# antao97/SegGroup

Hardware: AMD Instinct MI355X
Metric: pseudo-label scenes/sec (150k pts, 1.5k segs) (higher is better)
Workload: dtype f32 (fp32 accumulate; operands split into 2 x fp16 pieces on v_mfma_f32_32x32x16_f16; kNN / FPS scores in exact fp32 order); 1 GPU; 64 distinct synthetic scenes per GPU per step, 150000 pts / 1500 segs each (BASELINE.json configs[2]; configs[1] = the same scene shape, single scene); mode=ins_infer, scenes_in_flight=112, engine=14 groups x 8 scenes per batched launch, weights=tests/golden/weights_g2.npz, parallelism=scene-parallel x1

## Files before the change

### include/seggroup_hip.h

```cpp
#ifndef SEGGROUP_HIP_H
#define SEGGROUP_HIP_H

#include <stddef.h>
#include <stdint.h>

#ifdef __cplusplus
extern "C" {
#endif

#define SG_OK          0
#define SG_EINVAL     -1
#define SG_EHIP       -2
#define SG_ENOMEM     -3
#define SG_ESTALL     -4
#define SG_EUNSUP     -5

#define SG_MODE_INS_INFER 0
#define SG_MODE_SEM_INFER 1

#define SG_NUM_LABEL_VECTORS 14
#define SG_RANGE_WORDS 256
#define SG_MAX_POINTS (1 << 20)

const char* sg_last_error(void);
// ... 64 lines not shown
                          const int32_t* d_seg_off, const int32_t* d_seg_chunk_off, const float* d_segbox,
                          const float* d_chunk_box, const int32_t* d_slot_of_pos, int k, int pos0, int32_t* d_knn, void* stream);
int sg_knn_seed_points(const int32_t* d_knn, const int32_t* d_members, int N, int k, int32_t* d_seed, void* stream);
int sg_cluster_knn_seeded(const float* d_sxyzw, const int32_t* d_smpos, int N, const int32_t* d_cl_off,
                          const int32_t* d_tile_cl, const int32_t* d_tile_lo, const int32_t* d_tile_hi, int T,
                          const int32_t* d_cl_seg_off, const int32_t* d_order, const int32_t* d_dst,
                          const int32_t* d_seg_off, const int32_t* d_seg_chunk_off, const float* d_segbox,
                          const float* d_chunk_box, const int32_t* d_slot_of_pos, const int32_t* d_seed,
                          const int32_t* d_seg_prevcl, const int32_t* d_members, const float* d_point_rec,
                          int k, int pos0, int32_t* d_knn, void* stream);

int sg_knn_chunk_table(const int32_t* d_order, const int32_t* d_dst, const int32_t* d_seg_off, const int32_t* d_seg_chunk_off,
                       const float* d_chunk_box, int S, const int32_t* d_slot_chunk0, float* d_cc, void* stream);
int sg_cluster_knn_2pass(const float* d_sxyzw, const int32_t* d_smpos, int N, const int32_t* d_cl_off,
                         const int32_t* d_tile_cl, const int32_t* d_tile_lo, const int32_t* d_tile_hi,
                         const int32_t* d_tile_chunk0, int T, const int32_t* d_cl_chunk_off, const float* d_cc,
                         int k, int pos0, int32_t* d_knn, void* stream);
int sg_cluster_knn_sorted_w(const float* d_sxyzw, const int32_t* d_smpos, int N, const int32_t* d_cl_off,
                            const int32_t* d_tile_cl, const int32_t* d_tile_lo, const int32_t* d_tile_hi, int T,
                            const int32_t* d_cl_seg_off, const int32_t* d_order, const int32_t* d_dst,
                            const int32_t* d_seg_off, const int32_t* d_seg_chunk_off, const float* d_segbox,
                            const float* d_chunk_box, const int32_t* d_slot_of_pos, int k, int pos0, int waves_per_tile,
                            int32_t* d_knn, void* stream);

size_t sg_edgeconv_ws_bytes(int N);
int sg_edgeconv_forward(const float* d_x9m, const int32_t* d_knn, int N, int k, int layers,
                        const float* d_w1, const float* d_g1, const float* d_b1,
                        const float* d_w2, const float* d_g2, const float* d_b2,
                        float* d_out, void* d_ws, size_t ws_bytes, void* stream);
int sg_edgeconv_forward_r(const float* d_x9m, const int32_t* d_knn, int N, int k, int layers, const float* d_w1, const float* d_g1,
                          const float* d_b1, const float* d_w2, const float* d_g2, const float* d_b2, float* d_out, void* d_ws,
                          size_t ws_bytes, unsigned int* d_range_bits, void* stream);
#define SG_EDGECONV_COMPILER_LOOP 1u
int sg_edgeconv_forward_x(const float* d_x9m, const int32_t* d_knn, int N, int k, int layers, const float* d_w1, const float* d_g1,
                          const float* d_b1, const float* d_w2, const float* d_g2, const float* d_b2, float* d_out, void* d_ws,
                          size_t ws_bytes, unsigned int* d_range_bits, unsigned int flags, void* stream);
int sg_edge_range(const float* d_x9m, int N, unsigned int* d_range_bits, void* stream);

size_t sg_gcn_ws_bytes(int S, int D, int E);
int sg_gcn_forward(const float* d_x, int S, int D, const int32_t* d_adj, int E,
                   const int32_t* d_rowptr, const int32_t* d_col, const int32_t* d_eid,
                   const float* d_w, float alpha, float* d_out, void* d_ws, size_t ws_bytes, void* stream);

int sg_export_labels(const int32_t* d_unmap, int V, const int32_t* d_seg_of_point, int N,
                     const int32_t* d_tables, int T, int S, int32_t* d_out, void* stream);

// ... 292 lines not shown
```

### seggroup_amd/csrc/kernels_knn_sorted.hip

```cpp
#include <cstdlib>


#include "engine_ctx.h"
#include "knn_device.h"
#include "sg_common.h"
#include "wave_ops.h"

namespace {

using namespace sgknn;

#ifdef SG_KNN_PROFILE
constexpr bool kKnnProfile = true;
#else
constexpr bool kKnnProfile = false;
#endif

constexpr int kChunkPts = 32;
constexpr int kQuadS = 4;

__device__ inline unsigned int spread10(unsigned int v);
__device__ inline unsigned int morton30(const float* __restrict__ r, const float* __restrict__ b) {
    const float e[3] = {b[3] - b[0], b[4] - b[1], b[5] - b[2]};
    const float emax = fmaxf(fmaxf(e[0], e[1]), e[2]);
// ... 475 lines not shown
    const sg::SlotCtx& c = cx[blockIdx.y];
    if ((int)blockIdx.x >= c.lay_nbig) return;
    const int i = c.lay_big[2 * blockIdx.x], r0 = c.lay_big[2 * blockIdx.x + 1];
    layer_layout_body(c.data, c.seg_points, c.seg_off, c.sperm, c.order, c.dst, c.cl, c.cl_mean, c.members, nullptr, c.cluster_of_pos,
                      c.slot_of_pos, c.x9m, c.sxyzw, c.smpos, c.point_rec, c.seed_id, c.ec_range, i, r0, r0 + sg::kLayoutPiece);
}

__global__ void k_knn_operands(const float* __restrict__ data, const int32_t* __restrict__ seg_points,
                               const int32_t* __restrict__ seg_off, const int32_t* __restrict__ sperm,
                               const int32_t* __restrict__ order, const int32_t* __restrict__ dst,
                               float4* __restrict__ sxyzw, int32_t* __restrict__ smpos) {
    const int i = blockIdx.x;
    const int s = order[i];
    const int lo = seg_off[s], n = seg_off[s + 1] - lo, d = dst[i];
    for (int r = threadIdx.x; r < n; r += blockDim.x) {
        const int ci = sperm[lo + r];
        const float* row = data + (size_t)seg_points[ci] * 6;
        const float x = row[0], y = row[1], z = row[2];
        sxyzw[d + r] = make_float4(x, y, z, (x * x + y * y) + z * z);
        smpos[d + r] = d + (ci - lo);
    }
}

__device__ unsigned long long g_knn5_stats[16];
#ifdef SG_KNN_SELFCHECK
__device__ unsigned long long g_knn_check[8 + 128];
#endif

template <int K, int kSlices, bool kSeeded>
__device__ __forceinline__ void cluster_knn_sorted_body(
    sg::gptr<const float4> sxyzw, sg::gptr<const int32_t> smpos, sg::gptr<const int32_t> cl_off,
    sg::gptr<const int32_t> tile_cl, sg::gptr<const int32_t> tile_lo, sg::gptr<const int32_t> tile_hi,
    sg::gptr<const int32_t> cl_seg_off, sg::gptr<const int32_t> order, sg::gptr<const int32_t> dst,
    sg::gptr<const int32_t> seg_off, sg::gptr<const int32_t> seg_chunk_off, sg::gptr<const float> segbox,
    sg::gptr<const float> chunk_box, sg::gptr<const int32_t> slot_of_pos, int pos0, sg::gptr<int32_t> knn, int dbg_arg,
    sg::gptr<const int32_t> seed, sg::gptr<const int32_t> seg_prevcl, sg::gptr<const int32_t> members,
    sg::gptr<const float4> point_rec, int t, sg::gptr<int32_t> seed_out = nullptr) {
    static_assert(!kSeeded || kSlices == 1, "seeding is built for one wave per tile");
    const int dbg = kKnnProfile ? dbg_arg : 0;
    constexpr int kBufS = kSlices == 1 ? 12 : 20;
    constexpr int kSlotBatch = kSlices == 1 ? 32 : 128;
    static_assert(kSlices == 1 || kBufS >= K, "the merge area aliases the append buffers");
    __shared__ float4 slab[kSlices][kChunkPts + kQuadS];
    __shared__ int slab_i[kSlices][kChunkPts + kQuadS];
    __shared__ unsigned long long buf[kBufS][64 * kSlices];
    __shared__ unsigned int thr_pub[kSlices][64];
    __shared__ unsigned int thr5_pub[kSlices][64];
    __shared__ __attribute__((aligned(16))) float chunkbox_lds[kSlices][kSlices == 1 ? 256 : 64];
    __shared__ int st_m[kSlotBatch], st_c0[kSlotBatch], st_d[kSlotBatch], st_pc[kSlotBatch];
    __shared__ __attribute__((aligned(16))) float st_box[kSlotBatch][8];
    const int c = tile_cl[t];
    const int clo = cl_off[c], n = cl_off[c + 1] - clo;
    const int tid = threadIdx.x, lane = tid & 63, wave = tid >> 6;
    const int q = tile_lo[t] + lane;
    const bool active = q < tile_hi[t];
    const int myrow = active ? smpos[q] : 0;
    if (n <= K) {
        if (active && wave == 0) {
            int lane_e = lane;
            asm volatile("" : "+v"(lane_e));
            const int row_e = smpos[tile_lo[t] + lane_e];
            const sg::gptr<int32_t> o = knn + (size_t)row_e * K;
#pragma unroll
            for (int j = 0; j < K; ++j) o[j] = j < n ? clo + j : pos0;
            if (seed_out) {
                const sg::gptr<int32_t> so = seed_out + (size_t)members[row_e] * K;
#pragma unroll
                for (int j = 0; j < K; ++j) so[j] = members[j < n ? clo + j : pos0];
            }
        }
        return;
    }
    float4 me = make_float4(0.f, 0.f, 0.f, 0.f);
    if (active) me = sxyzw[q];
    double kv[K];
#pragma unroll
    for (int j = 0; j < K; ++j) kv[j] = list_empty();
    double thr_l = active ? list_empty() : to_list(~0ull);
    int myprev = -1;
    if (kSeeded && active) {
        myprev = seg_prevcl[order[slot_of_pos[myrow]]];
        if (myprev >= 0) {
            const sg::gptr<const int32_t> sp = seed + (size_t)members[myrow] * K;
#pragma unroll
            for (int j = 0; j < K; ++j) {
                const float4 rec = point_rec[sp[j]];
                kv[j] = to_list(make_key(score4(me, make_float4(rec.x, rec.y, rec.z, (rec.x * rec.x + rec.y * rec.y) + rec.z * rec.z)),
                                         __float_as_int(rec.w) - clo));
            }
            thr_l = kv[K - 1];
#ifdef SG_KNN_SELFCHECK
            bool bad_ = false;
#pragma unroll
            for (int j = 0; j + 1 < K; ++j) bad_ |= from_list(kv[j]) <= from_list(kv[j + 1]);
            if (bad_ && atomicAdd(&g_knn_check[0], 1ull) == 0ull) {
                for (int j = 0; j < K; ++j) {
                    const float4 rec = point_rec[sp[j]];
                    g_knn_check[8 + j] = ((unsigned long long)(unsigned)sp[j] << 32) | (unsigned)(__float_as_int(rec.w) - clo);
                    g_knn_check[8 + 20 + j] = from_list(kv[j]);
                    const float again = score4(me, make_float4(rec.x, rec.y, rec.z, (rec.x * rec.x + rec.y * rec.y) + rec.z * rec.z));
// ... 82 lines not shown
        const double use_l = best_thr();
        if ((dbg & 32) && lane == 0) atomicAdd(&g_knn5_stats[6], 1ull);
        if (!__any(ok && list_key(box_score_bound(me, bx), 0) >= use_l)) return;
        if ((dbg & 32) && lane == 0) atomicAdd(&g_knn5_stats[5], 1ull);
        if (dbg & 16) ++dbg_scanned;
        __builtin_amdgcn_wave_barrier();
        if (lane < kChunkPts + kQuadS) {
            const bool in = lane < m;
            float4 cand = make_float4(0.f, 0.f, 0.f, INFINITY);
            if (in) cand = sxyzw[p0 + lane];
            cw[lane] = cand;
            ci[lane] = in ? smpos[p0 + lane] - clo : 0x7fffffff;
        }
        __builtin_amdgcn_wave_barrier();
        float fbound = score_bound(list_max(use_l, thr_l), ok);
        for (int i = 0; i < m; i += kQuadS) {
            float4 c4[kQuadS];
#pragma unroll
            for (int u = 0; u < kQuadS; ++u) c4[u] = cw[i + u];
            float sc4[kQuadS];
#pragma unroll
            for (int u = 0; u < kQuadS; ++u) sc4[u] = score4(me, c4[u]);
            static_assert(kQuadS == 4, "the group test below is written for four candidates");
            if (fmaxf(fmaxf(sc4[0], sc4[1]), fmaxf(sc4[2], sc4[3])) >= fbound) {
#pragma unroll
                for (int u = 0; u < kQuadS; ++u) {
                    if (sc4[u] >= fbound) {
                        const double key = list_key(sc4[u], ci[i + u]);
                        if (key > use_l && key > thr_l) {
                            buf[cnt][tid] = (unsigned long long)__double_as_longlong(key);
                            ++cnt;
                        }
                    }
                }
            }
            if (__any(cnt > kBufS - kQuadS)) {
                drain();
                fbound = score_bound(list_max(use_l, thr_l), ok);
            }
        }
    };
    const int so0 = cl_seg_off[c], nslots = cl_seg_off[c + 1] - so0;
    const int own = slot_of_pos[active ? myrow : smpos[tile_lo[t]]] - so0;
    const int own0 = __shfl(own, 0);
    auto slot_of = [&](int r) {
        int sl = own0 + r;
        if (sl >= nslots) sl -= nslots;
        return so0 + sl;
    };
    float* cbx = &chunkbox_lds[wave][0];
    float qlo[3] = {0.f, 0.f, 0.f}, qhi[3] = {0.f, 0.f, 0.f}, qw = 0.f;
    if (kSlices == 1) {
        const float4 m0 = active ? me : make_float4(sgw::bcast(me.x, 0), sgw::bcast(me.y, 0), sgw::bcast(me.z, 0), sgw::bcast(me.w, 0));
        qlo[0] = sgw::wave_min(m0.x); qlo[1] = sgw::wave_min(m0.y); qlo[2] = sgw::wave_min(m0.z);
        qhi[0] = sgw::wave_max(m0.x); qhi[1] = sgw::wave_max(m0.y); qhi[2] = sgw::wave_max(m0.z);
        qw = sgw::wave_max(m0.w);
    }
    auto ring_chunk = [](int start, int e, int nch, bool two_sided) {
        int ch = start + (two_sided ? ((e & 1) ? -((e + 1) >> 1) : (e >> 1)) : e);
        if (ch >= nch) ch -= nch;
        if (ch < 0) ch += nch;
        return ch;
    };
    auto scan_segment = [&](int sg_m, int sg_c0, int d, const float* sbox, int pc, int& item, int start, bool two_sided = false) {
        const int nch = (sg_m + kChunkPts - 1) / kChunkPts;
        const double use_l = best_thr();
        if (kSeeded) ok = pc < 0 || pc != myprev;
        if ((dbg & 32) && lane == 0 && wave == 0) atomicAdd(&g_knn5_stats[7], 1ull);
        if (!__any(ok && list_key(box_score_bound(me, sbox), 0) >= use_l)) { item += nch; return; }
        if constexpr (kSlices == 1) {
            for (int j0 = 0; j0 < nch; j0 += 32) {
                const int nb = min(32, nch - j0);
                const int mych = ring_chunk(start, min(j0 + lane, nch - 1), nch, two_sided);
                bool pass = lane < nb;
                float weakest = -INFINITY;
                if (nch > 16) {
                    const unsigned int o = list_score(best_thr());
                    float mine = INFINITY;
                    if (active && ok) mine = o < 0x00800000u ? -INFINITY : __uint_as_float((o & 0x80000000u) ? (o ^ 0x80000000u) : ~o);
                    weakest = sgw::wave_min(mine);
                }
                __builtin_amdgcn_wave_barrier();
                if (lane < nb) {
                    const sg::gptr<const float4> bp = (sg::gptr<const float4>)(chunk_box + (size_t)(sg_c0 + mych) * 8);
                    const float4 b0 = bp[0], b1 = bp[1];
                    reinterpret_cast<float4*>(cbx)[2 * lane] = b0;
                    reinterpret_cast<float4*>(cbx)[2 * lane + 1] = b1;
                    if (nch > 16) {
                        const float gx = fmaxf(fmaxf(b0.x - qhi[0], qlo[0] - b0.w), 0.f);
                        const float gy = fmaxf(fmaxf(b0.y - qhi[1], qlo[1] - b1.x), 0.f);
                        const float gz = fmaxf(fmaxf(b0.z - qhi[2], qlo[2] - b1.y), 0.f);
                        pass = -((gx * gx + gy * gy) + gz * gz) * 0.999999f + 9.6e-7f * (qw + b1.z) >= weakest;
                    }
                }
                __builtin_amdgcn_wave_barrier();
                unsigned long long live = __ballot(pass);
                while (live) {
                    const int j = __ffsll((unsigned long long)live) - 1;
                    live &= live - 1;
                    const int ch = ring_chunk(start, j0 + j, nch, two_sided);
                    scan_chunk(cbx + j * 8, d + ch * kChunkPts, min(kChunkPts, sg_m - ch * kChunkPts));
                }
            }
            item += nch;
            return;
        }
        for (int j0 = 0; j0 < nch; j0 += 8) {
            const int nb = min(8, nch - j0);
            __builtin_amdgcn_wave_barrier();
            if (lane < nb * 8) cbx[lane] = chunk_box[(size_t)(sg_c0 + j0) * 8 + lane];
            __builtin_amdgcn_wave_barrier();
// ... 24 lines not shown
            const int slot = slot_of(r0 + e), sg = order[slot];
            st_m[e] = seg_off[sg + 1] - seg_off[sg];
            st_c0[e] = seg_chunk_off[sg];
            st_d[e] = dst[slot];
            if (kSeeded) st_pc[e] = seg_prevcl[sg];
            const sg::gptr<const float4> bp = (sg::gptr<const float4>)(segbox + (size_t)sg * 8);
            reinterpret_cast<float4*>(&st_box[e][0])[0] = bp[0];
            reinterpret_cast<float4*>(&st_box[e][0])[1] = bp[1];
        }
        __syncthreads();
        for (int i = 0; i < nb; ++i) scan_segment(st_m[i], st_c0[i], st_d[i], &st_box[i][0], kSeeded ? st_pc[i] : -1, item, 0);
    }
    drain();
    const unsigned long long t3 = (dbg & 16) ? __builtin_readcyclecounter() : 0ull;
#ifdef SG_KNN_SELFCHECK
    if (kSeeded && active) {
        bool bad_ = false;
#pragma unroll
        for (int j = 0; j + 1 < K; ++j) bad_ |= from_list(kv[j]) <= from_list(kv[j + 1]);
        if (bad_) atomicAdd(&g_knn_check[1], 1ull);
    }
#endif
    if (kSlices == 1) {
        if (active) {
            int lane_o = lane;
            asm volatile("" : "+v"(lane_o));
            const int row_o = smpos[tile_lo[t] + lane_o];
            const sg::gptr<int32_t> o = knn + (size_t)row_o * K;
#pragma unroll
            for (int j = 0; j < K; ++j) o[j] = clo + list_index(kv[j]);
            if (seed_out) {
                const sg::gptr<int32_t> so = seed_out + (size_t)members[row_o] * K;
#pragma unroll
                for (int j = 0; j < K; ++j) so[j] = members[clo + list_index(kv[j])];
            }
        }
    } else {
        __syncthreads();
        unsigned long long* lists = &buf[0][0];
    #pragma unroll
        for (int j = 0; j < K; ++j) lists[((size_t)wave * K + j) * 64 + lane] = from_list(kv[j]);
        __syncthreads();
        if (wave == 0 && active) {
            int p[kSlices];
            unsigned long long h[kSlices];
    #pragma unroll
            for (int w = 0; w < kSlices; ++w) { p[w] = 0; h[w] = lists[((size_t)w * K) * 64 + lane]; }
            const sg::gptr<int32_t> o = knn + (size_t)myrow * K;
            for (int j = 0; j < K; ++j) {
                int bw = 0;
                unsigned long long bk = h[0];
    #pragma unroll
                for (int w = 1; w < kSlices; ++w) if (h[w] > bk) { bk = h[w]; bw = w; }
                o[j] = clo + key_index(bk);
    #pragma unroll
                for (int w = 0; w < kSlices; ++w)
                    if (w == bw) { ++p[w]; h[w] = p[w] < K ? lists[((size_t)w * K + p[w]) * 64 + lane] : 0ull; }
            }
        }
    }
    if ((dbg & 16) && lane == 0) {
        const unsigned long long t4 = __builtin_readcyclecounter();
        if (wave == 0) atomicAdd(&g_knn5_stats[0], 1ull);
        atomicAdd(&g_knn5_stats[1], t1 - t0);
        atomicAdd(&g_knn5_stats[2], t2 - t1);
        atomicAdd(&g_knn5_stats[3], t3 - t2);
        atomicAdd(&g_knn5_stats[4], t4 - t3);
        atomicMax(&g_knn5_stats[13], (min(t4 - t0, 0xffffffull) << 40) | ((unsigned long long)min(n >> 6, 0x3fff) << 26) |
                                     ((unsigned long long)min(nslots, 0xfff) << 14) | (unsigned long long)min(dbg_scanned, 0x3fff));
        if (n > 2048) { atomicAdd(&g_knn5_stats[14], t4 - t0); atomicAdd(&g_knn5_stats[15], 1ull); }
    }
}
template <int K, int kSlices, bool kSeeded = false>
__global__ __launch_bounds__(64 * kSlices, kSlices == 1 ? 4 : 1) void k_cluster_knn_sorted(
    const float4* __restrict__ sxyzw, const int32_t* __restrict__ smpos, const int32_t* __restrict__ cl_off,
    const int32_t* __restrict__ tile_cl, const int32_t* __restrict__ tile_lo, const int32_t* __restrict__ tile_hi,
    const int32_t* __restrict__ cl_seg_off, const int32_t* __restrict__ order, const int32_t* __restrict__ dst,
    const int32_t* __restrict__ seg_off, const int32_t* __restrict__ seg_chunk_off, const float* __restrict__ segbox,
    const float* __restrict__ chunk_box, const int32_t* __restrict__ slot_of_pos, int pos0, int32_t* __restrict__ knn, int dbg_arg,
    const int32_t* __restrict__ seed = nullptr, const int32_t* __restrict__ seg_prevcl = nullptr, const int32_t* __restrict__ members = nullptr,
    const float4* __restrict__ point_rec = nullptr) {
    using sg::as_global;
    cluster_knn_sorted_body<K, kSlices, kSeeded>(as_global(sxyzw), as_global(smpos), as_global(cl_off), as_global(tile_cl), as_global(tile_lo),
                                                 as_global(tile_hi), as_global(cl_seg_off), as_global(order), as_global(dst), as_global(seg_off),
                                                 as_global(seg_chunk_off), as_global(segbox), as_global(chunk_box), as_global(slot_of_pos), pos0,
                                                 as_global(knn), dbg_arg, as_global(seed), as_global(seg_prevcl), as_global(members),
                                                 as_global(point_rec), blockIdx.x);
}
template <int K, int kSlices, bool kSeeded>
__global__ __launch_bounds__(64 * kSlices, kSlices == 1 ? 4 : 1) void k_cluster_knn_sorted_b(const sg::SlotCtx* __restrict__ cx, int write_seed) {
    const sg::SlotCtx& c = cx[blockIdx.x];
    if ((int)blockIdx.y >= c.T) return;
    using sg::as_global;
    cluster_knn_sorted_body<K, kSlices, kSeeded>(as_global(c.sxyzw), as_global(c.smpos), as_global(c.cl_pt_off), as_global(c.tile_cl),
                                                 as_global(c.tile_lo), as_global(c.tile_hi), as_global(c.cl_seg_off), as_global(c.order),
                                                 as_global(c.dst), as_global(c.seg_off), as_global(c.seg_chunk_off), as_global(c.segbox),
                                                 as_global(c.chunk_box), as_global(c.slot_of_pos), c.pos0, as_global(c.knn), 0,
                                                 as_global(c.knn_seed), as_global(c.seg_prevcl), as_global(c.seed_id), as_global(c.point_rec),
                                                 blockIdx.y, kSlices == 1 && !kSeeded && write_seed ? as_global(c.knn_seed) : nullptr);
}


__global__ void k_knn_seed_points(const int32_t* __restrict__ knn, const int32_t* __restrict__ members, int N, int K,
                                  int32_t* __restrict__ seed) {
    const int i = blockIdx.x * blockDim.x + threadIdx.x;
    if (i >= N * K) return;
    seed[(size_t)members[i / K] * K + i % K] = members[knn[i]];
}
__global__ void k_knn_seed_points_b(const sg::SlotCtx* __restrict__ cx) {
    const sg::SlotCtx& c = cx[blockIdx.y];
    const int i = blockIdx.x * blockDim.x + threadIdx.x;
    if (i >= c.N * 20) return;
    c.knn_seed[(size_t)c.seed_id[i / 20] * 20 + i % 20] = c.seed_id[c.knn[i]];
}

template <int K>
__device__ inline void score_insert(float (&sv)[K], float x) {
#pragma unroll
    for (int j = K - 1; j > 0; --j) sv[j] = __builtin_amdgcn_fmed3f(sv[j - 1], sv[j], x);
    sv[0] = fmaxf(sv[0], x);
}

// ... 156 lines not shown
                 const unsigned long long key = make_key(sc, idx);
                 if (key > thr) {
                     buf[cnt][lane] = key;
                     ++cnt;
                 }
             },
             [&]() { return __any(cnt > kBuf2 - kQuadS - 1); }, drain);
    }
    if (active) {
        int32_t* o = knn + (size_t)myrow * K;
#pragma unroll
        for (int j = 0; j < K; ++j) o[j] = clo + key_index(kv[j]);
    }
    if ((dbg & 16) && lane == 0) {
        const unsigned long long t2 = __builtin_readcyclecounter();
        atomicAdd(&g_knn5_stats[0], 1ull);
        atomicAdd(&g_knn5_stats[1], t1 - t0);
        atomicAdd(&g_knn5_stats[3], t2 - t1);
    }
}

}

int sg::knn_variant_for(int T, int override) {
    if (override == 0 || override == 1 || override == 2 || override == 4 || override == 8) return override;
    return T >= 2048 ? 8 : T >= 1024 ? 2 : 4;
}

namespace sg {

bool sort_boxes_fits_lds(int max_seg) { return max_seg <= kSortCap; }

int b_sort_boxes(const SlotCtx* d_ctx, const BatchDims& bd, hipStream_t st, int which) {
    if (bd.nslots == 0 || bd.max_S == 0) return SG_OK;
    if (which & 1) k_segment_sort_boxes_b<<<dim3(bd.max_S, bd.nslots), 256, 0, st>>>(d_ctx);
    if ((which & 2) && bd.max_big > 0) {
        const int wins = sg::cdiv(bd.max_N, kWin);
        k_bigseg_box_b<<<dim3(bd.max_big * kBigPieces, bd.nslots), kPieceBlock, 0, st>>>(d_ctx);
        k_bigseg_keys_b<<<dim3(bd.max_big * kBigPieces, bd.nslots), kPieceBlock, 0, st>>>(d_ctx);
        k_bigseg_scatter_b<<<dim3(bd.max_big * kBigPieces, bd.nslots), kPieceBlock, 0, st>>>(d_ctx);
        k_bigseg_runs_b<<<dim3(wins, bd.nslots), kBigBlock, 0, st>>>(d_ctx);
        k_bigseg_boxes_b<<<dim3(wins, bd.nslots), 512, 0, st>>>(d_ctx);
    }
    SG_LAUNCH_CHECK();
    return SG_OK;
}

int b_layer_layout(const SlotCtx* d_ctx, const BatchDims& bd, hipStream_t st) {
    if (bd.nslots == 0 || bd.max_S == 0) return SG_OK;
    k_layer_layout_b<<<dim3(bd.max_S, bd.nslots), 256, 0, st>>>(d_ctx);
    if (bd.max_lay_big > 0) k_layer_layout_big_b<<<dim3(bd.max_lay_big, bd.nslots), 256, 0, st>>>(d_ctx);
    SG_LAUNCH_CHECK();
    return SG_OK;
}

int b_cluster_knn(const SlotCtx* d_ctx, const BatchDims& bd, int waves_per_tile, bool seeded, hipStream_t st, bool write_seed, bool* wrote_seed) {
    if (wrote_seed) *wrote_seed = false;
    if (bd.nslots == 0 || bd.max_T == 0) return SG_OK;
    if (bd.max_N > sgknn::kListMaxPoints) return sg::fail(SG_EUNSUP, "in-cluster kNN: %d points in a scene, the list keys carry 20 index bits (N <= %d)", bd.max_N, sgknn::kListMaxPoints);
    const dim3 grid(bd.nslots, bd.max_T);
    if (seeded) k_cluster_knn_sorted_b<20, 1, true><<<grid, 64, 0, st>>>(d_ctx, 0);
    else if (waves_per_tile == 1) {
        k_cluster_knn_sorted_b<20, 1, false><<<grid, 64, 0, st>>>(d_ctx, write_seed ? 1 : 0);
        if (wrote_seed) *wrote_seed = write_seed;
    } else if (waves_per_tile == 2) k_cluster_knn_sorted_b<20, 2, false><<<grid, 128, 0, st>>>(d_ctx, 0);
    else k_cluster_knn_sorted_b<20, 4, false><<<grid, 256, 0, st>>>(d_ctx, 0);
    SG_LAUNCH_CHECK();
    return SG_OK;
}

int b_knn_seed_points(const SlotCtx* d_ctx, const BatchDims& bd, hipStream_t st) {
    if (bd.nslots == 0 || bd.max_N == 0) return SG_OK;
    k_knn_seed_points_b<<<dim3(sg::cdiv((long long)bd.max_N * 20, 256), bd.nslots), 256, 0, st>>>(d_ctx);
    SG_LAUNCH_CHECK();
    return SG_OK;
}

}

#ifdef SG_KNN_PROFILE
static int g_knn5_dbg = getenv("SG_KNN_DEBUG") ? atoi(getenv("SG_KNN_DEBUG")) : 0;
#else
static constexpr int g_knn5_dbg = 0;
#endif

extern "C" {

#ifdef SG_KNN_PROFILE
int sg_debug_knn5_stats(unsigned long long* h_out) {
    SG_HIP(hipMemcpyFromSymbol(h_out, HIP_SYMBOL(g_knn5_stats), sizeof(unsigned long long) * 16));
    unsigned long long z[16] = {0};
    SG_HIP(hipMemcpyToSymbol(HIP_SYMBOL(g_knn5_stats), z, sizeof z));
    return SG_OK;
}
#endif

#ifdef SG_KNN_SELFCHECK
int sg_debug_knn_check(unsigned long long* h_out) {
    SG_HIP(hipMemcpyFromSymbol(h_out, HIP_SYMBOL(g_knn_check), sizeof(unsigned long long) * 136));
    unsigned long long z[136] = {0};
    SG_HIP(hipMemcpyToSymbol(HIP_SYMBOL(g_knn_check), z, sizeof z));
    return SG_OK;
}
#endif

size_t sg_segment_sort_ws_bytes(int N) { return sg::align_up((size_t)std::max(N, 1) * 16, 64) + bigseg_scratch_slots(std::max(N, 1)) * sizeof(BigScratch) + 64; }

int sg_layer_layout(const float* d_data, int N, const int32_t* d_seg_points, const int32_t* d_seg_off, const int32_t* d_sperm, int S,
                    const int32_t* d_order, const int32_t* d_dst, const int32_t* d_cl, const float* d_cl_mean, int32_t* d_members,
                    int32_t* d_pos_of_point, int32_t* d_cluster_of_pos, int32_t* d_slot_of_pos, float* d_x9m, float* d_sxyzw,
                    int32_t* d_smpos, float* d_point_rec, int32_t* d_seed_id, unsigned int* d_range_bits, void* stream) {
    SG_REQUIRE(N >= 0 && S >= 0 && d_sperm && d_cl_mean && d_members && d_pos_of_point && d_cluster_of_pos && d_slot_of_pos && d_x9m &&
                   d_sxyzw && d_smpos, "sg_layer_layout: bad arguments");
    if (S == 0) return SG_OK;
// ... 78 lines not shown
    SG_REQUIRE(N < (1 << 25), "sg_cluster_knn_2pass: sorted positions are packed in 25 bits (N < 2^25)");
    if (k != 20) return sg::fail(SG_EUNSUP, "sg_cluster_knn_2pass: only k == 20 is built (model.py:788,829), got %d", k);
    if (T == 0) return SG_OK;
    k_cluster_knn_2pass<20><<<T, 64, 0, sg::as_stream(stream)>>>(reinterpret_cast<const float4*>(d_sxyzw), d_smpos, d_cl_off, d_tile_cl,
                                                                 d_tile_lo, d_tile_hi, d_tile_chunk0, d_cl_chunk_off,
                                                                 reinterpret_cast<const float4*>(d_cc), pos0, d_knn, g_knn5_dbg);
    SG_LAUNCH_CHECK();
    return SG_OK;
}

int sg_cluster_knn_sorted_w(const float* d_sxyzw, const int32_t* d_smpos, int N, const int32_t* d_cl_off, const int32_t* d_tile_cl,
                            const int32_t* d_tile_lo, const int32_t* d_tile_hi, int T, const int32_t* d_cl_seg_off,
                            const int32_t* d_order, const int32_t* d_dst, const int32_t* d_seg_off, const int32_t* d_seg_chunk_off,
                            const float* d_segbox, const float* d_chunk_box, const int32_t* d_slot_of_pos, int k, int pos0,
                            int waves_per_tile, int32_t* d_knn, void* stream) {
    SG_REQUIRE(N >= 0 && T >= 0 && d_knn && d_sxyzw && d_smpos, "sg_cluster_knn_sorted: bad arguments");
    SG_REQUIRE(N <= sgknn::kListMaxPoints, "sg_cluster_knn_sorted: the list keys carry 20 index bits (N <= 2^20)");
    if (k != 20) return sg::fail(SG_EUNSUP, "sg_cluster_knn_sorted: only k == 20 is built (model.py:788,829), got %d", k);
    if (T == 0) return SG_OK;
    const int slices = (waves_per_tile == 1 || waves_per_tile == 2 || waves_per_tile == 4) ? waves_per_tile : (T >= 2048 ? 1 : T >= 1024 ? 2 : 4);
#define SG_KNN_LAUNCH(S)                                                                                                  \
    k_cluster_knn_sorted<20, S><<<T, 64 * S, 0, sg::as_stream(stream)>>>(                                                 \
        reinterpret_cast<const float4*>(d_sxyzw), d_smpos, d_cl_off, d_tile_cl, d_tile_lo, d_tile_hi, d_cl_seg_off, d_order, d_dst, \
        d_seg_off, d_seg_chunk_off, d_segbox, d_chunk_box, d_slot_of_pos, pos0, d_knn, g_knn5_dbg)
    if (slices == 1) SG_KNN_LAUNCH(1);
    else if (slices == 2) SG_KNN_LAUNCH(2);
    else SG_KNN_LAUNCH(4);
#undef SG_KNN_LAUNCH
    SG_LAUNCH_CHECK();
    return SG_OK;
}

int sg_cluster_knn_sorted(const float* d_sxyzw, const int32_t* d_smpos, int N, const int32_t* d_cl_off, const int32_t* d_tile_cl,
                          const int32_t* d_tile_lo, const int32_t* d_tile_hi, int T, const int32_t* d_cl_seg_off,
                          const int32_t* d_order, const int32_t* d_dst, const int32_t* d_seg_off, const int32_t* d_seg_chunk_off,
                          const float* d_segbox, const float* d_chunk_box, const int32_t* d_slot_of_pos, int k, int pos0,
                          int32_t* d_knn, void* stream) {
    return sg_cluster_knn_sorted_w(d_sxyzw, d_smpos, N, d_cl_off, d_tile_cl, d_tile_lo, d_tile_hi, T, d_cl_seg_off, d_order, d_dst, d_seg_off,
                                   d_seg_chunk_off, d_segbox, d_chunk_box, d_slot_of_pos, k, pos0, 0, d_knn, stream);
}

}
```

### seggroup_amd/csrc/knn_device.h

```cpp
#pragma once
#include <hip/hip_runtime.h>

namespace sgknn {

__device__ inline float score4(const float4& me, const float4& p) {
    const float tt = __builtin_fmaf(me.z, p.z, __builtin_fmaf(me.y, p.y, me.x * p.x));
    const float inner = -2.0f * tt;
    return ((-p.w) - inner) - me.w;
}

__device__ inline unsigned long long make_key(float score, int idx) {
    const unsigned int u = __float_as_uint(score);
    const unsigned int o = u ^ ((u >> 31) ? 0xffffffffu : 0x80000000u);
    return ((unsigned long long)o << 32) | (unsigned int)(0xffffffffu - (unsigned int)idx);
}
__device__ inline int key_index(unsigned long long key) { return (int)(0xffffffffu - (unsigned int)(key & 0xffffffffu)); }

__device__ __forceinline__ unsigned int sel_mask(unsigned int if_clear, unsigned int if_set, unsigned long long mask) {
    unsigned int r;
    asm("v_cndmask_b32_e64 %0, %1, %2, %3" : "=v"(r) : "v"(if_clear), "v"(if_set), "s"(mask));
    return r;
}
template <int K>
__device__ inline void key_insert(unsigned long long (&kv)[K], unsigned long long x) {
// ... 6 lines not shown
        const unsigned int pl = (unsigned int)kv[j - 1], ph = (unsigned int)(kv[j - 1] >> 32);
        const unsigned int ol = (unsigned int)kv[j], oh = (unsigned int)(kv[j] >> 32);
        const unsigned int tl = sel_mask(xl, pl, c[j - 1]), th = sel_mask(xh, ph, c[j - 1]);
        kv[j] = ((unsigned long long)sel_mask(oh, th, c[j]) << 32) | sel_mask(ol, tl, c[j]);
    }
    kv[0] = ((unsigned long long)sel_mask((unsigned int)(kv[0] >> 32), xh, c[0]) << 32) | sel_mask((unsigned int)kv[0], xl, c[0]);
}

constexpr int kListIndexBits = 20;
constexpr int kListMaxPoints = 1 << kListIndexBits;
__device__ __forceinline__ double list_empty() { return __hiloint2double(0x43300000, 0); }
__device__ __forceinline__ double to_list(unsigned long long key) {
    const unsigned int o = (unsigned int)(key >> 32), lo = (unsigned int)key;
    return __hiloint2double((int)(0x43300000u | (o >> 12)), (int)((o << 20) | (lo & 0xfffffu)));
}
__device__ __forceinline__ unsigned long long from_list(double d) {
    const unsigned int hi = (unsigned int)__double2hiint(d), lo = (unsigned int)__double2loint(d);
    return ((unsigned long long)((hi << 12) | (lo >> 20)) << 32) | (0xfff00000u | lo);
}
__device__ __forceinline__ double list_key(float score, int idx) {
    const unsigned int u = __float_as_uint(score);
    const unsigned int o = u ^ ((u >> 31) ? 0xffffffffu : 0x80000000u);
    return __hiloint2double((int)(0x43300000u | (o >> 12)), (int)((o << 20) | (~(unsigned int)idx & 0xfffffu)));
}
__device__ __forceinline__ unsigned int list_score(double d) {
    return __builtin_amdgcn_alignbit((unsigned int)__double2hiint(d), (unsigned int)__double2loint(d), 20);
}
__device__ __forceinline__ double list_floor(unsigned int o) {
    return __longlong_as_double(__double_as_longlong(__hiloint2double((int)(0x43300000u | (o >> 12)), (int)(o << 20))) - 1ll);
}
__device__ __forceinline__ int list_index(double d) { return (int)(0xfffffu - ((unsigned int)__double2loint(d) & 0xfffffu)); }
__device__ __forceinline__ double list_max(double a, double b) { double r; asm("v_max_f64 %0, %1, %2" : "=v"(r) : "v"(a), "v"(b)); return r; }
__device__ __forceinline__ double list_min(double a, double b) { double r; asm("v_min_f64 %0, %1, %2" : "=v"(r) : "v"(a), "v"(b)); return r; }
template <int K>
__device__ __forceinline__ void list_insert_l(double (&kv)[K], double x) {
#pragma unroll
    for (int j = K - 1; j > 0; --j) kv[j] = list_max(kv[j], list_min(kv[j - 1], x));
    kv[0] = list_max(kv[0], x);
}
template <int K>
__device__ __forceinline__ void list_insert(double (&kv)[K], unsigned long long key) {
    const double x = to_list(key);
#pragma unroll
    for (int j = K - 1; j > 0; --j) kv[j] = list_max(kv[j], list_min(kv[j - 1], x));
    kv[0] = list_max(kv[0], x);
}
// ... 40 lines not shown
```

### seggroup_amd/hip.py

```python
from __future__ import annotations

import contextlib
import ctypes as C
import os
from typing import Optional

_HERE = os.path.dirname(os.path.abspath(__file__))
LIB_PATH = os.environ.get("SEGGROUP_HIP_LIB") or os.path.join(_HERE, "libseggroup_hip.so")
HOST_LIB_OVERRIDE = os.environ.get("SEGGROUP_HIP_HOST_LIB")

SG_OK, SG_EINVAL, SG_EHIP, SG_ENOMEM, SG_ESTALL, SG_EUNSUP = 0, -1, -2, -3, -4, -5
MODE_INS_INFER, MODE_SEM_INFER = 0, 1
COLOUR_SEMANTIC, COLOUR_INSTANCE, COLOUR_SEGMENT, COLOUR_GROUPING = 0, 1, 2, 3
NUM_LABEL_VECTORS = 14
LABEL_NAMES = [f"layer_{l}.{k}" for l in (1, 2, 3, 4) for k in ("seg", "ins", "sem")] + ["final.ins", "final.sem"]

c_f32p = C.POINTER(C.c_float)
c_i32p = C.POINTER(C.c_int32)
c_i64p = C.POINTER(C.c_int64)
c_u8p = C.POINTER(C.c_uint8)
vp = C.c_void_p


class SgError(RuntimeError):
# ... 9 lines not shown

class Scene(C.Structure):
    _fields_ = [("N", C.c_int), ("S", C.c_int), ("E0", C.c_int), ("V", C.c_int),
                ("d_data", vp), ("d_adj", vp), ("d_seg_of_point", vp), ("d_seg_points", vp), ("d_seg_off", vp),
                ("d_unmap", vp), ("d_gt", vp),
                ("h_seg_first", vp), ("h_seg_size", vp), ("h_seg_ins", vp), ("h_seg_sem", vp), ("h_seg_of_vertex", vp)]


class Result(C.Structure):
    _fields_ = [("h_labels", vp), ("iou_sem", C.c_float * 80), ("iou_ins", C.c_float * 80), ("acc", C.c_float * 4),
                ("trace", C.c_int32 * 5), ("stalled", C.c_int32), ("used_fallback", C.c_int32), ("h_tables", vp)]


class Classifier(C.Structure):
    _fields_ = [(n, vp) for n in ("w1", "gamma", "beta", "w2", "b2")]


class Debug(C.Structure):
    _fields_ = [("d_samples1", vp), ("d_feat1", vp), ("d_pointfeat", vp * 2), ("d_knn", vp * 2), ("d_members", vp * 2),
                ("h_gcn", vp * 2), ("h_dist", vp * 3), ("h_adj", vp * 4), ("n_adj", C.c_int32 * 4),
                ("h_feat5", vp), ("h_ins5", vp), ("h_sem5", vp), ("n5", C.c_int32), ("tape", vp), ("d_cat", vp * 2)]


_I, _Z = C.c_int, C.c_size_t
SIGNATURES = {
    "sg_last_error": (C.c_char_p, []),
    "sg_version": (_I, []),
    "sg_device_count": (_I, []),
    "sg_selftest_wave_ops": (_I, [C.POINTER(C.c_int), vp]),
    "sg_selftest_list_insert": (_I, [C.POINTER(C.c_int), vp]),
    "sg_contract_ws_bytes": (_Z, [_I]),
    "sg_contract_point_edges": (_I, [vp, _I, vp, _I, _I, vp, _I, vp, vp, _Z, vp]),
    "sg_gather_members": (_I, [vp, vp, _I, vp, vp, vp, vp, vp, vp, vp, vp]),
    "sg_fps_ws_bytes": (_Z, [_I]),
    "sg_fps_sample": (_I, [vp, _I, _I, vp, vp, _I, _I, _I, _I, vp, vp, vp, _Z, vp]),
    "sg_mlp1_ws_bytes": (_Z, [_I]),
    "sg_mlp1_forward": (_I, [vp, _I, vp, vp, vp, vp, _I, vp, _Z, vp]),
    "sg_edge_distance": (_I, [vp, _I, _I, vp, _I, vp, vp]),
    "sg_group_max_rows": (_I, [vp, _I, _I, vp, vp, _I, vp, _I, vp]),
    "sg_segment_max": (_I, [vp, _I, _I, vp, vp, _I, _I, vp]),
    "sg_center_ws_bytes": (_Z, [_I, _I]),
    "sg_center_clusters": (_I, [vp, _I, vp, vp, _I, vp, vp, vp, _I, vp, vp, vp, vp, _Z, vp]),
    "sg_cluster_knn": (_I, [vp, _I, vp, vp, vp, vp, _I, _I, _I, vp, vp]),
    "sg_segment_boxes": (_I, [vp, vp, vp, _I, vp, vp]),
    "sg_cluster_knn_pruned": (_I, [vp, _I, vp, vp, vp, vp, _I, vp, vp, vp, vp, vp, vp, _I, _I, vp, vp]),
    "sg_segment_sort_ws_bytes": (_Z, [_I]),
    "sg_knn_operands": (_I, [vp, vp, vp, vp, _I, vp, vp, vp, vp, vp]),
    "sg_cluster_knn_sorted": (_I, [vp, vp, _I, vp, vp, vp, vp, _I, vp, vp, vp, vp, vp, vp, vp, vp, _I, _I, vp, vp]),
    "sg_segment_sort_boxes": (_I, [vp, _I, vp, vp, vp, _I, vp, _I, vp, vp, vp, vp, vp, _Z, vp]),
    "sg_layer_layout": (_I, [vp, _I, vp, vp, vp, _I, vp, vp, vp, vp, vp, vp, vp, vp, vp, vp, vp, vp, vp, vp, vp]),
    "sg_cluster_knn_sorted_w": (_I, [vp, vp, _I, vp, vp, vp, vp, _I, vp, vp, vp, vp, vp, vp, vp, vp, _I, _I, _I, vp, vp]),
    "sg_knn_seed_points": (_I, [vp, vp, _I, _I, vp, vp]),
    "sg_cluster_knn_seeded": (_I, [vp, vp, _I, vp, vp, vp, vp, _I, vp, vp, vp, vp, vp, vp, vp, vp, vp, vp, vp, vp, _I, _I, vp, vp]),
    "sg_knn_chunk_table": (_I, [vp, vp, vp, vp, vp, _I, vp, vp, vp]),
    "sg_cluster_knn_2pass": (_I, [vp, vp, _I, vp, vp, vp, vp, vp, _I, vp, vp, _I, _I, vp, vp]),
    "sg_nearest_point_ws_bytes": (_Z, [_I]),
    "sg_nearest_point": (_I, [vp, _I, vp, _I, _I, vp, vp, _Z, vp]),
    "sg_prep_sample_ws_bytes": (_Z, [_I, _I]),
    "sg_prep_sample_points": (_I, [vp, vp, _I, vp, _I, vp, vp, C.POINTER(C.c_int), vp, _Z, vp]),
    "sg_pointcloud_adjacency_ws_bytes": (_Z, [_I, _I]),
    "sg_pointcloud_adjacency": (_I, [vp, _I, _I, _I, vp, C.POINTER(C.c_int), vp, _Z, vp]),
    "sg_mesh_adjacency_ws_bytes": (_Z, [_I]),
    "sg_mesh_adjacency": (_I, [vp, _I, vp, _I, vp, C.POINTER(C.c_int), vp, C.POINTER(C.c_int), vp, _Z, vp]),
    "sg_segment_lists_ws_bytes": (_Z, [_I, _I]),
    "sg_segment_lists": (_I, [vp, _I, vp, _I, vp, vp, vp, C.POINTER(C.c_int), vp, _Z, vp]),
    "sg_write_seg_json": (_I, [C.c_char_p, vp, vp, _I, _I]),
    "sg_train_tail_ws_bytes": (_Z, [_I, _I]),
    "sg_train_tail_forward": (_I, [vp, _I, vp, _I, vp, vp, vp, vp, vp, vp, _Z, vp]),
    "sg_train_tail_backward": (_I, [_I, _I, vp, vp, vp, C.c_float, vp, vp, vp, vp, vp, vp, vp, _Z, vp]),
    "sg_group_mean_rows": (_I, [vp, _I, _I, vp, vp, _I, vp, _I, vp]),
    "sg_fps_general_ws_bytes": (C.c_size_t, [_I]),
    "sg_fps_general": (_I, [vp, _I, _I, _I, _I, _I, vp, vp, vp, C.c_size_t, vp]),
    "sg_knn_general": (_I, [vp, _I, _I, _I, _I, vp, vp]),
    "sg_group_max_rows_backward": (_I, [vp, _I, _I, vp, vp, _I, vp, _I, vp, _I, vp]),
# ... 127 lines not shown
            _runtime = C.CDLL(c, mode=C.RTLD_GLOBAL)
            return _runtime
        except OSError as e:
            err = e
    raise RuntimeError(f"no HIP runtime (libamdhip64.so) could be loaded: {err}")


def lib() -> C.CDLL:
    global _lib
    if _lib is None:
        path = HOST_LIB_OVERRIDE or LIB_PATH
        if not os.path.exists(path):
            raise RuntimeError(
                f"{path} is missing: build it with `python -c 'import __graft_entry__ as g; g.build()'` "
                "(or `make -C seggroup_amd/csrc`).  The SegGroup hot path has no CPU fallback.")
        _load_hip_runtime()
        l = C.CDLL(path)
        for name, (res, args) in SIGNATURES.items():
            try:
                fn = getattr(l, name)
            except AttributeError:
                if HOST_LIB_OVERRIDE:
                    continue
                raise
            fn.restype = res
            fn.argtypes = args
        _lib = l
    return _lib


_roctx = None


@contextlib.contextmanager
def roctx_range(name: str):
    global _roctx
    if not os.environ.get("SG_ROCTX"):
        yield
        return
    if _roctx is None:
        _roctx = False
        for cand in ("librocprofiler-sdk-roctx.so", "/opt/rocm/lib/librocprofiler-sdk-roctx.so", "libroctx64.so"):
            try:
                _roctx = C.CDLL(cand, mode=C.RTLD_GLOBAL)
                break
            except OSError:
# ... 29 lines not shown
```

Before: 3502 scenes/s.

## Add dense brute-force kNN path for small clusters, skipping chunk pruning

For clusters with at most a threshold number of points (default 256, env-tunable), the single-wave kNN kernel now scans every candidate in groups of twelve through a shared-memory slab and merges straight into the top-20 list, bypassing the segment/chunk box pruning machinery. The query tile bounding box is now computed lazily and stored in LDS only when chunk pruning actually needs it. This targets the bookkeeping overhead of the pruned search on small clusters, at the cost of exhaustive distance work for clusters near the threshold. A standalone entry point and profiling counters are also added.

Result: no change. 3519 scenes/s, median of 3 (+0.5%).

```diff
diff --git a/include/seggroup_hip.h b/include/seggroup_hip.h
--- a/include/seggroup_hip.h
+++ b/include/seggroup_hip.h
@@ -110,6 +110,13 @@
                             const int32_t* d_seg_off, const int32_t* d_seg_chunk_off, const float* d_segbox,
                             const float* d_chunk_box, const int32_t* d_slot_of_pos, int k, int pos0, int waves_per_tile,
                             int32_t* d_knn, void* stream);
+int sg_knn_dense_max(void);
+int sg_cluster_knn_sorted_d(const float* d_sxyzw, const int32_t* d_smpos, int N, const int32_t* d_cl_off,
+                            const int32_t* d_tile_cl, const int32_t* d_tile_lo, const int32_t* d_tile_hi, int T,
+                            const int32_t* d_cl_seg_off, const int32_t* d_order, const int32_t* d_dst,
+                            const int32_t* d_seg_off, const int32_t* d_seg_chunk_off, const float* d_segbox,
+                            const float* d_chunk_box, const int32_t* d_slot_of_pos, int k, int pos0, int dense_max,
+                            const int32_t* d_members, int32_t* d_seed_out, int32_t* d_knn, void* stream);
 
 size_t sg_edgeconv_ws_bytes(int N);
 int sg_edgeconv_forward(const float* d_x9m, const int32_t* d_knn, int N, int k, int layers,
diff --git a/seggroup_amd/csrc/kernels_knn_sorted.hip b/seggroup_amd/csrc/kernels_knn_sorted.hip
--- a/seggroup_amd/csrc/kernels_knn_sorted.hip
+++ b/seggroup_amd/csrc/kernels_knn_sorted.hip
@@ -521,7 +521,8 @@
     }
 }
 
-__device__ unsigned long long g_knn5_stats[16];
+constexpr int kKnnStats = 24;
+__device__ unsigned long long g_knn5_stats[kKnnStats];
 #ifdef SG_KNN_SELFCHECK
 __device__ unsigned long long g_knn_check[8 + 128];
 #endif
@@ -534,7 +535,7 @@
     sg::gptr<const int32_t> seg_off, sg::gptr<const int32_t> seg_chunk_off, sg::gptr<const float> segbox,
     sg::gptr<const float> chunk_box, sg::gptr<const int32_t> slot_of_pos, int pos0, sg::gptr<int32_t> knn, int dbg_arg,
     sg::gptr<const int32_t> seed, sg::gptr<const int32_t> seg_prevcl, sg::gptr<const int32_t> members,
-    sg::gptr<const float4> point_rec, int t, sg::gptr<int32_t> seed_out = nullptr) {
+    sg::gptr<const float4> point_rec, int t, sg::gptr<int32_t> seed_out = nullptr, int dense_max = 0) {
     static_assert(!kSeeded || kSlices == 1, "seeding is built for one wave per tile");
     const int dbg = kKnnProfile ? dbg_arg : 0;
     constexpr int kBufS = kSlices == 1 ? 12 : 20;
@@ -548,6 +549,7 @@
     __shared__ __attribute__((aligned(16))) float chunkbox_lds[kSlices][kSlices == 1 ? 256 : 64];
     __shared__ int st_m[kSlotBatch], st_c0[kSlotBatch], st_d[kSlotBatch], st_pc[kSlotBatch];
     __shared__ __attribute__((aligned(16))) float st_box[kSlotBatch][8];
+    __shared__ __attribute__((aligned(16))) float qbox_lds[8];
     const int c = tile_cl[t];
     const int clo = cl_off[c], n = cl_off[c + 1] - clo;
     const int tid = threadIdx.x, lane = tid & 63, wave = tid >> 6;
@@ -575,6 +577,54 @@
     double kv[K];
 #pragma unroll
     for (int j = 0; j < K; ++j) kv[j] = list_empty();
+    auto emit_rows = [&]() {
+        if (active) {
+            int lane_o = lane;
+            asm volatile("" : "+v"(lane_o));
+            const int row_o = smpos[tile_lo[t] + lane_o];
+            const sg::gptr<int32_t> o = knn + (size_t)row_o * K;
+#pragma unroll
+            for (int j = 0; j < K; ++j) o[j] = clo + list_index(kv[j]);
+            if (seed_out) {
+                const sg::gptr<int32_t> so = seed_out + (size_t)members[row_o] * K;
+#pragma unroll
+                for (int j = 0; j < K; ++j) so[j] = members[clo + list_index(kv[j])];
+            }
+        }
+    };
+    if constexpr (K == 20 && kSlices == 1 && !kSeeded) {
+        if (n <= dense_max) {
+            static_assert(kChunkPts + kQuadS == 36, "the dense path fills the slab with three groups of twelve");
+            float4* dw = slab[0];
+            int* di = slab_i[0];
+            const int ngroups = (n + 11) / 12;
+            if ((dbg & 32) && lane == 0) { atomicAdd(&g_knn5_stats[16], 1ull); atomicAdd(&g_knn5_stats[17], (unsigned long long)ngroups); }
+            int r12 = 0;
+            for (int g = 0; g < ngroups; ++g) {
+                if (r12 == 0) {
+                    __builtin_amdgcn_wave_barrier();
+                    if (lane < kChunkPts + kQuadS) {
+                        const int p = g * 12 + lane;
+                        float4 cand = make_float4(0.f, 0.f, 0.f, INFINITY);
+                        int bits = 0;
+                        if (p < n) { cand = sxyzw[clo + p]; bits = ~(smpos[clo + p] - clo) & 0xfffff; }
+                        dw[lane] = cand;
+                        di[lane] = bits;
+                    }
+                    __builtin_amdgcn_wave_barrier();
+                }
+                const int left = n - g * 12;
+                double b[12];
+#pragma unroll
+                for (int u = 0; u < 12; ++u)
+                    b[u] = list_key_bits(score4(me, dw[r12 + u]), (unsigned int)di[r12 + u], u < left ? 0xffffffffu : 0u);
+                list_merge12(kv, b);
+                r12 = r12 == 24 ? 0 : r12 + 12;
+            }
+            emit_rows();
+            return;
+        }
+    }
     double thr_l = active ? list_empty() : to_list(~0ull);
     int myprev = -1;
     if (kSeeded && active) {
@@ -703,6 +753,12 @@
 #pragma unroll
             for (int u = 0; u < kQuadS; ++u) sc4[u] = score4(me, c4[u]);
             static_assert(kQuadS == 4, "the group test below is written for four candidates");
+            if (dbg & 32) {
+                int took = 0;
+#pragma unroll
+                for (int u = 0; u < kQuadS; ++u) took += (i + u < m && __any(sc4[u] >= fbound)) ? 1 : 0;
+                if (lane == 0) { atomicAdd(&g_knn5_stats[18], (unsigned long long)min(kQuadS, m - i)); atomicAdd(&g_knn5_stats[19], (unsigned long long)took); }
+            }
             if (fmaxf(fmaxf(sc4[0], sc4[1]), fmaxf(sc4[2], sc4[3])) >= fbound) {
 #pragma unroll
                 for (int u = 0; u < kQuadS; ++u) {
@@ -730,13 +786,18 @@
         return so0 + sl;
     };
     float* cbx = &chunkbox_lds[wave][0];
-    float qlo[3] = {0.f, 0.f, 0.f}, qhi[3] = {0.f, 0.f, 0.f}, qw = 0.f;
-    if (kSlices == 1) {
+    bool have_qbox = false;
+    auto tile_qbox = [&]() {
         const float4 m0 = active ? me : make_float4(sgw::bcast(me.x, 0), sgw::bcast(me.y, 0), sgw::bcast(me.z, 0), sgw::bcast(me.w, 0));
-        qlo[0] = sgw::wave_min(m0.x); qlo[1] = sgw::wave_min(m0.y); qlo[2] = sgw::wave_min(m0.z);
-        qhi[0] = sgw::wave_max(m0.x); qhi[1] = sgw::wave_max(m0.y); qhi[2] = sgw::wave_max(m0.z);
-        qw = sgw::wave_max(m0.w);
-    }
+        const float lo0 = sgw::wave_min(m0.x), lo1 = sgw::wave_min(m0.y), lo2 = sgw::wave_min(m0.z);
+        const float hi0 = sgw::wave_max(m0.x), hi1 = sgw::wave_max(m0.y), hi2 = sgw::wave_max(m0.z);
+        const float w = sgw::wave_max(m0.w);
+        if (lane == 0) {
+            reinterpret_cast<float4*>(qbox_lds)[0] = make_float4(lo0, lo1, lo2, w);
+            reinterpret_cast<float4*>(qbox_lds)[1] = make_float4(hi0, hi1, hi2, 0.f);
+        }
+        have_qbox = true;
+    };
     auto ring_chunk = [](int start, int e, int nch, bool two_sided) {
         int ch = start + (two_sided ? ((e & 1) ? -((e + 1) >> 1) : (e >> 1)) : e);
         if (ch >= nch) ch -= nch;
@@ -756,6 +817,7 @@
                 bool pass = lane < nb;
                 float weakest = -INFINITY;
                 if (nch > 16) {
+                    if (!have_qbox) tile_qbox();
                     const unsigned int o = list_score(best_thr());
                     float mine = INFINITY;
                     if (active && ok) mine = o < 0x00800000u ? -INFINITY : __uint_as_float((o & 0x80000000u) ? (o ^ 0x80000000u) : ~o);
@@ -768,6 +830,8 @@
                     reinterpret_cast<float4*>(cbx)[2 * lane] = b0;
                     reinterpret_cast<float4*>(cbx)[2 * lane + 1] = b1;
                     if (nch > 16) {
+                        const float4 ql = reinterpret_cast<const float4*>(qbox_lds)[0], qh = reinterpret_cast<const float4*>(qbox_lds)[1];
+                        const float qlo[3] = {ql.x, ql.y, ql.z}, qhi[3] = {qh.x, qh.y, qh.z}, qw = ql.w;
                         const float gx = fmaxf(fmaxf(b0.x - qhi[0], qlo[0] - b0.w), 0.f);
                         const float gy = fmaxf(fmaxf(b0.y - qhi[1], qlo[1] - b1.x), 0.f);
                         const float gz = fmaxf(fmaxf(b0.z - qhi[2], qlo[2] - b1.y), 0.f);
@@ -838,19 +902,7 @@
     }
 #endif
     if (kSlices == 1) {
-        if (active) {
-            int lane_o = lane;
-            asm volatile("" : "+v"(lane_o));
-            const int row_o = smpos[tile_lo[t] + lane_o];
-            const sg::gptr<int32_t> o = knn + (size_t)row_o * K;
-#pragma unroll
-            for (int j = 0; j < K; ++j) o[j] = clo + list_index(kv[j]);
-            if (seed_out) {
-                const sg::gptr<int32_t> so = seed_out + (size_t)members[row_o] * K;
-#pragma unroll
-                for (int j = 0; j < K; ++j) so[j] = members[clo + list_index(kv[j])];
-            }
-        }
+        emit_rows();
     } else {
         __syncthreads();
         unsigned long long* lists = &buf[0][0];
@@ -895,16 +947,16 @@
     const int32_t* __restrict__ seg_off, const int32_t* __restrict__ seg_chunk_off, const float* __restrict__ segbox,
     const float* __restrict__ chunk_box, const int32_t* __restrict__ slot_of_pos, int pos0, int32_t* __restrict__ knn, int dbg_arg,
     const int32_t* __restrict__ seed = nullptr, const int32_t* __restrict__ seg_prevcl = nullptr, const int32_t* __restrict__ members = nullptr,
-    const float4* __restrict__ point_rec = nullptr) {
+    const float4* __restrict__ point_rec = nullptr, int32_t* __restrict__ seed_out = nullptr, int dense_max = 0) {
     using sg::as_global;
     cluster_knn_sorted_body<K, kSlices, kSeeded>(as_global(sxyzw), as_global(smpos), as_global(cl_off), as_global(tile_cl), as_global(tile_lo),
                                                  as_global(tile_hi), as_global(cl_seg_off), as_global(order), as_global(dst), as_global(seg_off),
                                                  as_global(seg_chunk_off), as_global(segbox), as_global(chunk_box), as_global(slot_of_pos), pos0,
                                                  as_global(knn), dbg_arg, as_global(seed), as_global(seg_prevcl), as_global(members),
-                                                 as_global(point_rec), blockIdx.x);
+                                                 as_global(point_rec), blockIdx.x, as_global(seed_out), dense_max);
 }
 template <int K, int kSlices, bool kSeeded>
-__global__ __launch_bounds__(64 * kSlices, kSlices == 1 ? 4 : 1) void k_cluster_knn_sorted_b(const sg::SlotCtx* __restrict__ cx, int write_seed) {
+__global__ __launch_bounds__(64 * kSlices, kSlices == 1 ? 4 : 1) void k_cluster_knn_sorted_b(const sg::SlotCtx* __restrict__ cx, int write_seed, int dense_max) {
     const sg::SlotCtx& c = cx[blockIdx.x];
     if ((int)blockIdx.y >= c.T) return;
     using sg::as_global;
@@ -913,7 +965,7 @@
                                                  as_global(c.dst), as_global(c.seg_off), as_global(c.seg_chunk_off), as_global(c.segbox),
                                                  as_global(c.chunk_box), as_global(c.slot_of_pos), c.pos0, as_global(c.knn), 0,
                                                  as_global(c.knn_seed), as_global(c.seg_prevcl), as_global(c.seed_id), as_global(c.point_rec),
-                                                 blockIdx.y, kSlices == 1 && !kSeeded && write_seed ? as_global(c.knn_seed) : nullptr);
+                                                 blockIdx.y, kSlices == 1 && !kSeeded && write_seed ? as_global(c.knn_seed) : nullptr, dense_max);
 }
 
 
@@ -1116,6 +1168,12 @@
 
 }
 
+constexpr int kDenseMax = 256;
+static const int g_knn_dense_max = [] {
+    const char* e = getenv("SG_KNN_DENSE_MAX");
+    return e ? std::max(0, atoi(e)) : kDenseMax;
+}();
+
 int sg::knn_variant_for(int T, int override) {
     if (override == 0 || override == 1 || override == 2 || override == 4 || override == 8) return override;
     return T >= 2048 ? 8 : T >= 1024 ? 2 : 4;
@@ -1153,12 +1211,12 @@
     if (bd.nslots == 0 || bd.max_T == 0) return SG_OK;
     if (bd.max_N > sgknn::kListMaxPoints) return sg::fail(SG_EUNSUP, "in-cluster kNN: %d points in a scene, the list keys carry 20 index bits (N <= %d)", bd.max_N, sgknn::kListMaxPoints);
     const dim3 grid(bd.nslots, bd.max_T);
-    if (seeded) k_cluster_knn_sorted_b<20, 1, true><<<grid, 64, 0, st>>>(d_ctx, 0);
+    if (seeded) k_cluster_knn_sorted_b<20, 1, true><<<grid, 64, 0, st>>>(d_ctx, 0, 0);
     else if (waves_per_tile == 1) {
-        k_cluster_knn_sorted_b<20, 1, false><<<grid, 64, 0, st>>>(d_ctx, write_seed ? 1 : 0);
+        k_cluster_knn_sorted_b<20, 1, false><<<grid, 64, 0, st>>>(d_ctx, write_seed ? 1 : 0, g_knn_dense_max);
         if (wrote_seed) *wrote_seed = write_seed;
-    } else if (waves_per_tile == 2) k_cluster_knn_sorted_b<20, 2, false><<<grid, 128, 0, st>>>(d_ctx, 0);
-    else k_cluster_knn_sorted_b<20, 4, false><<<grid, 256, 0, st>>>(d_ctx, 0);
+    } else if (waves_per_tile == 2) k_cluster_knn_sorted_b<20, 2, false><<<grid, 128, 0, st>>>(d_ctx, 0, 0);
+    else k_cluster_knn_sorted_b<20, 4, false><<<grid, 256, 0, st>>>(d_ctx, 0, 0);
     SG_LAUNCH_CHECK();
     return SG_OK;
 }
@@ -1182,8 +1240,8 @@
 
 #ifdef SG_KNN_PROFILE
 int sg_debug_knn5_stats(unsigned long long* h_out) {
-    SG_HIP(hipMemcpyFromSymbol(h_out, HIP_SYMBOL(g_knn5_stats), sizeof(unsigned long long) * 16));
-    unsigned long long z[16] = {0};
+    SG_HIP(hipMemcpyFromSymbol(h_out, HIP_SYMBOL(g_knn5_stats), sizeof(unsigned long long) * kKnnStats));
+    unsigned long long z[kKnnStats] = {0};
     SG_HIP(hipMemcpyToSymbol(HIP_SYMBOL(g_knn5_stats), z, sizeof z));
     return SG_OK;
 }
@@ -1308,11 +1366,32 @@
 #define SG_KNN_LAUNCH(S)                                                                                                  \
     k_cluster_knn_sorted<20, S><<<T, 64 * S, 0, sg::as_stream(stream)>>>(                                                 \
         reinterpret_cast<const float4*>(d_sxyzw), d_smpos, d_cl_off, d_tile_cl, d_tile_lo, d_tile_hi, d_cl_seg_off, d_order, d_dst, \
-        d_seg_off, d_seg_chunk_off, d_segbox, d_chunk_box, d_slot_of_pos, pos0, d_knn, g_knn5_dbg)
+        d_seg_off, d_seg_chunk_off, d_segbox, d_chunk_box, d_slot_of_pos, pos0, d_knn, g_knn5_dbg, nullptr, nullptr, nullptr, nullptr, nullptr, \
+        S == 1 ? g_knn_dense_max : 0)
     if (slices == 1) SG_KNN_LAUNCH(1);
     else if (slices == 2) SG_KNN_LAUNCH(2);
     else SG_KNN_LAUNCH(4);
 #undef SG_KNN_LAUNCH
+    SG_LAUNCH_CHECK();
+    return SG_OK;
+}
+
+int sg_knn_dense_max(void) { return g_knn_dense_max; }
+
+int sg_cluster_knn_sorted_d(const float* d_sxyzw, const int32_t* d_smpos, int N, const int32_t* d_cl_off, const int32_t* d_tile_cl,
+                            const int32_t* d_tile_lo, const int32_t* d_tile_hi, int T, const int32_t* d_cl_seg_off,
+                            const int32_t* d_order, const int32_t* d_dst, const int32_t* d_seg_off, const int32_t* d_seg_chunk_off,
+                            const float* d_segbox, const float* d_chunk_box, const int32_t* d_slot_of_pos, int k, int pos0,
+                            int dense_max, const int32_t* d_members, int32_t* d_seed_out, int32_t* d_knn, void* stream) {
+    SG_REQUIRE(N >= 0 && T >= 0 && d_knn && d_sxyzw && d_smpos, "sg_cluster_knn_sorted_d: bad arguments");
+    SG_REQUIRE(!d_seed_out || d_members, "sg_cluster_knn_sorted_d: the seed table needs the position -> id map (d_members)");
+    SG_REQUIRE(N <= sgknn::kListMaxPoints, "sg_cluster_knn_sorted_d: the list keys carry 20 index bits (N <= 2^20)");
+    if (k != 20) return sg::fail(SG_EUNSUP, "sg_cluster_knn_sorted_d: only k == 20 is built (model.py:788,829), got %d", k);
+    if (T == 0) return SG_OK;
+    k_cluster_knn_sorted<20, 1><<<T, 64, 0, sg::as_stream(stream)>>>(
+        reinterpret_cast<const float4*>(d_sxyzw), d_smpos, d_cl_off, d_tile_cl, d_tile_lo, d_tile_hi, d_cl_seg_off, d_order, d_dst,
+        d_seg_off, d_seg_chunk_off, d_segbox, d_chunk_box, d_slot_of_pos, pos0, d_knn, g_knn5_dbg, nullptr, nullptr, d_members, nullptr,
+        d_seed_out, dense_max < 0 ? g_knn_dense_max : dense_max);
     SG_LAUNCH_CHECK();
     return SG_OK;
 }
diff --git a/seggroup_amd/csrc/knn_device.h b/seggroup_amd/csrc/knn_device.h
--- a/seggroup_amd/csrc/knn_device.h
+++ b/seggroup_amd/csrc/knn_device.h
@@ -52,6 +52,11 @@
     const unsigned int u = __float_as_uint(score);
     const unsigned int o = u ^ ((u >> 31) ? 0xffffffffu : 0x80000000u);
     return __hiloint2double((int)(0x43300000u | (o >> 12)), (int)((o << 20) | (~(unsigned int)idx & 0xfffffu)));
+}
+__device__ __forceinline__ double list_key_bits(float score, unsigned int idx_bits, unsigned int keep) {
+    const unsigned int u = __float_as_uint(score);
+    const unsigned int o = (u ^ ((u >> 31) ? 0xffffffffu : 0x80000000u)) & keep;
+    return __hiloint2double((int)(0x43300000u | (o >> 12)), (int)((o << 20) | idx_bits));
 }
 __device__ __forceinline__ unsigned int list_score(double d) {
     return __builtin_amdgcn_alignbit((unsigned int)__double2hiint(d), (unsigned int)__double2loint(d), 20);
diff --git a/seggroup_amd/hip.py b/seggroup_amd/hip.py
--- a/seggroup_amd/hip.py
+++ b/seggroup_amd/hip.py
@@ -55,6 +55,7 @@
                 ("h_feat5", vp), ("h_ins5", vp), ("h_sem5", vp), ("n5", C.c_int32), ("tape", vp), ("d_cat", vp * 2)]
 
 
+_NEWER_SYMBOLS = ("sg_knn_dense_max", "sg_cluster_knn_sorted_d")
 _I, _Z = C.c_int, C.c_size_t
 SIGNATURES = {
     "sg_last_error": (C.c_char_p, []),
@@ -83,6 +84,8 @@
     "sg_segment_sort_boxes": (_I, [vp, _I, vp, vp, vp, _I, vp, _I, vp, vp, vp, vp, vp, _Z, vp]),
     "sg_layer_layout": (_I, [vp, _I, vp, vp, vp, _I, vp, vp, vp, vp, vp, vp, vp, vp, vp, vp, vp, vp, vp, vp, vp]),
     "sg_cluster_knn_sorted_w": (_I, [vp, vp, _I, vp, vp, vp, vp, _I, vp, vp, vp, vp, vp, vp, vp, vp, _I, _I, _I, vp, vp]),
+    "sg_knn_dense_max": (_I, []),
+    "sg_cluster_knn_sorted_d": (_I, [vp, vp, _I, vp, vp, vp, vp, _I, vp, vp, vp, vp, vp, vp, vp, vp, _I, _I, _I, vp, vp, vp, vp]),
     "sg_knn_seed_points": (_I, [vp, vp, _I, _I, vp, vp]),
     "sg_cluster_knn_seeded": (_I, [vp, vp, _I, vp, vp, vp, vp, _I, vp, vp, vp, vp, vp, vp, vp, vp, vp, vp, vp, vp, _I, _I, vp, vp]),
     "sg_knn_chunk_table": (_I, [vp, vp, vp, vp, vp, _I, vp, vp, vp]),
@@ -256,6 +259,8 @@
             except AttributeError:
                 if HOST_LIB_OVERRIDE:
                     continue
+                if os.environ.get("SEGGROUP_HIP_LIB") and name in _NEWER_SYMBOLS:
+                    continue
                 raise
             fn.restype = res
             fn.argtypes = args
```
